# Audio-WestlakeU/FS-EEND

Measured on AMD Instinct MI355X. Metric: audio frames/sec (T=500 chunks), higher is better.
Workload: dtype bf16

## Files before the change

### fs-eend_amd/csrc/api.hip

```cpp
#include "../../include/eend_hip.h"
#include "kernels.h"
#include <stdlib.h>
#include <string.h>

namespace {
GemmParams base_params(const void* A, int lda, const void* W, int ldw, const float* bias, int M, int N, int K) {
    GemmParams p;
    memset(&p, 0, sizeof(p));
    p.A = A; p.lda = lda; p.W = W; p.ldw = ldw; p.bias = bias;
    p.M = M; p.N = N; p.K = K; p.ldo = N; p.Tp = 64; p.H = 4; p.dh = 64; p.C = 1;
    p.alpha = 1.0f; p.eps = 1e-5f; p.conv_cin = 64; p.conv_pad = 0; p.drop.scale = 1.0f;
#ifdef EEND_GEMM_ABLATE
    const char* d = getenv("EEND_GEMM_DBG");
    p.dbg = d ? atoi(d) : 0;
#endif
    return p;
}

hipStream_t hs(void* stream) { return (hipStream_t)stream; }

bool linear_takes_proj(int act, const float* bias, int ldw, int ldo, int N, int K) {
    return act == 0 && K == 256 && ldw == 256 && bias && (N % 256) == 0 && N <= 1024 && (ldo & 7) == 0;
}
bool heads_shape_ok(int nseq, int Tp, int H, int dh) {
// ... 708 lines not shown
int eend_inproj_attn_packed_elems(void) { return (int)eend_inproj_attn_packed_nelems(); }

int eend_inproj_attn_pack_f16(const void* W_in, void* packed_out, void* stream) {
    return eend_launch_inproj_attn_pack(W_in, packed_out, (hipStream_t)stream);
}

int eend_inproj_attn_causal_packed_f16(const void* X_f16, int ldx, const void* W_packed, const float* b_in, void* O_f16,
                                       int nseq, int H, int Tp, int ldo, int mask_delay, int kv_len, void* stream) {
    if (!X_f16 || !W_packed || !b_in || !O_f16 || nseq > 16383) return EEND_EINVAL;
    InprojAttnParams p;
    p.X = X_f16; p.ldx = ldx; p.W = W_packed; p.bias = b_in; p.O = O_f16;
    p.nseq = nseq; p.H = H; p.Tp = Tp; p.ldo = ldo; p.mask_delay = mask_delay; p.kv_len = kv_len;
    return eend_launch_inproj_attn_stream(p, (hipStream_t)stream);
}

int eend_inproj_attn_long_scratch_elems(int nseq, int Tp, int mask_delay, int kv_len, long long* part_f16_elems, long long* lse_f32_elems) {
    if (!part_f16_elems || !lse_f32_elems) return EEND_EINVAL;
    long a = 0, b = 0;
    const int rc = eend_inproj_attn_long_scratch(nseq, Tp, mask_delay, kv_len, &a, &b);
    *part_f16_elems = a; *lse_f32_elems = b;
    return rc;
}

int eend_inproj_attn_causal_long_f16(const void* X_f16, int ldx, const void* W_packed, const float* b_in, void* O_f16, void* part_f16,
                                     float* lse_f32, int nseq, int H, int Tp, int ldo, int mask_delay, int kv_len, void* stream) {
    if (!X_f16 || !W_packed || !b_in || !O_f16 || !lse_f32 || nseq > 16383) return EEND_EINVAL;
    InprojAttnParams p;
    memset(&p, 0, sizeof(p));
    p.X = X_f16; p.ldx = ldx; p.W = W_packed; p.bias = b_in; p.O = O_f16; p.Opart = part_f16; p.lse = lse_f32;
    p.nseq = nseq; p.H = H; p.Tp = Tp; p.ldo = ldo; p.mask_delay = mask_delay; p.kv_len = kv_len;
// ... 168 lines not shown
```

### fs-eend_amd/csrc/attn_stream.hip

```cpp
#include "flash_tile.h"
#include "kernels.h"
#include "wstream.h"
#include <stdlib.h>

namespace {

constexpr int KB = 64;
constexpr int TILE = KB * 128;
constexpr int NW = 8;
constexpr int OSTG = 32 * 128;
constexpr int TP = 512;
constexpr int NT = TP / KB;
constexpr int WITEM = 16384;
constexpr int NITEM = 6;
constexpr int L_K = 0, L_V = NT * TILE, L_X = 2 * NT * TILE;
constexpr int SMEM = L_X + NW * OSTG;

DEV u32x2 pack_bf16x4(const f32x4 v) {
    bf16x4 o;
    o[0] = (__bf16)v[0]; o[1] = (__bf16)v[1]; o[2] = (__bf16)v[2]; o[3] = (__bf16)v[3];
    return __builtin_bit_cast(u32x2, o);
}

__global__ void inproj_attn_pack_kernel(const _Float16* __restrict__ W, _Float16* __restrict__ out) {
// ... 3 lines not shown
        const int pfrag = w >> 6, l = w & 63, f = l & 15, g = l >> 4, ks = pfrag >> 1, hf = pfrag & 1;
        const _Float16* src = W + (size_t)((n >> 1) * 256 + h * 64 + ((n & 1) * 2 + hf) * 16 + f) * 256 + ks * 32 + g * 8;
        _Float16* dst = out + (size_t)t * 8;
#pragma unroll
        for (int e = 0; e < 8; ++e) dst[e] = src[e];
    }
}

#ifdef EEND_AS_TRACE
__device__ unsigned long long g_as_trace[256 * 6 * 12];
#define AS_STAMP(k) do { ts[k] = __builtin_amdgcn_s_memtime(); } while (0)
#else
#define AS_STAMP(k) do {} while (0)
#endif

template <bool LONG, bool TRAIN = false, bool FULL = false>
__global__ __launch_bounds__(512)
void inproj_attn_stream_kernel(const InprojAttnParams p) {
    static_assert(!(LONG && TRAIN), "the training form covers windows up to 512 frames");
    static_assert(!(LONG && FULL), "groups of a long window have their own lengths");
    extern __shared__ __attribute__((aligned(16))) char smem[];
    char* Ks = smem + L_K;
    char* Vs = smem + L_V;
    char* Xs = smem + L_X;

    int tid = threadIdx.x;
    int lane = tid & 63;
    const int wave = __builtin_amdgcn_readfirstlane(tid >> 6);
    int frow = lane & 15, fkg = lane >> 4;
    const int nsh = p.nseq * 4;
    const int nitems = LONG ? nsh * p.npairs : nsh;
    const bool xcd_map = (p.nseq & 7) == 0 && ((gridDim.x & 7) == 0 || (int)gridDim.x >= nitems);
    auto item_of = [&](int L, int& seq_, int& h_) __attribute__((always_inline)) {
        if (xcd_map) {
            const int xcd = L & 7, slot = L >> 3;
            seq_ = (slot >> 2) * 8 + xcd; h_ = slot & 3;
        } else {
            seq_ = L >> 2; h_ = L & 3;
        }
    };
    int nblk = FULL ? 16 : p.Tp >> 5;
    int b1 = FULL ? wave : (wave < (nblk >> 1) ? wave : nblk + 2 * (wave - (nblk >> 1)));
    int b2 = FULL ? 15 - wave : (wave < (nblk >> 1) ? nblk - 1 - wave : b1 + 1);
    int qoff = 0, koff = 0, Tq = p.Tp, Tk = p.Tp, dl = p.mask_delay, kvl = p.kv_len, pair = 0;
    bool offd = false;
    auto tokbase = [&](int jt) __attribute__((always_inline)) { return jt < 2 ? 32 * b1 + 16 * jt : 32 * b2 + 16 * (jt - 2); };
    char* Ow = Xs + wave * OSTG;
    auto relaunder = [&]() __attribute__((always_inline)) {
        asm volatile("" : "+v"(tid));
        lane = tid & 63; frow = lane & 15; fkg = lane >> 4;
    };

    u32x4 xr[4][8];
    auto request_x = [&](int seq_, auto KEYS) __attribute__((always_inline)) {
        constexpr bool keys = decltype(KEYS)::value;
        const __amdgpu_buffer_rsrc_t rx = __builtin_amdgcn_make_buffer_rsrc((void*)((const _Float16*)p.X + ((size_t)seq_ * p.Tp + (keys ? koff : qoff)) * p.ldx), 0,
                                                                            (keys ? Tk : Tq) * p.ldx * 2, 0x00020000);
#pragma unroll
        for (int jt = 0; jt < 4; ++jt) {
// ... 6 lines not shown
    for (int item = blockIdx.x; item < nitems; item += gridDim.x) {
    int seq, h;
    if constexpr (LONG) {
        pair = item / nsh;
        item_of(item - pair * nsh, seq, h);
        const int qg = p.pq[pair], kg = p.pk[pair];
        qoff = qg * TP; koff = kg * TP;
        Tq = p.Tp - qoff < TP ? p.Tp - qoff : TP;
        Tk = p.Tp - koff < TP ? p.Tp - koff : TP;
        offd = qg != kg;
        dl = p.mask_delay + (qoff - koff);
        kvl = p.kv_len - koff < Tk ? p.kv_len - koff : Tk;
        nblk = Tq >> 5;
        b1 = wave < (nblk >> 1) ? wave : nblk + 2 * (wave - (nblk >> 1));
        b2 = wave < (nblk >> 1) ? nblk - 1 - wave : b1 + 1;
    } else {
        item_of(item, seq, h);
    }
    relaunder();
    request_x(seq, std::false_type{});
    asm volatile("s_waitcnt lgkmcnt(0)\n\ts_barrier" ::: "memory");
#ifdef EEND_AS_TRACE
    unsigned long long ts[12];
    const int tix = (item - (int)blockIdx.x) / (int)gridDim.x;
#endif
    AS_STAMP(0);

    u32x2 qpk[4][4];
    {
        const __amdgpu_buffer_rsrc_t rw = __builtin_amdgcn_make_buffer_rsrc((void*)((const char*)p.W + (size_t)h * NITEM * WITEM), 0,
                                                                            NITEM * WITEM, 0x00020000);
        f32x4 bq4[4];
        float bv1[4];
        f32x4 bk4[TRAIN ? 4 : 1], bv4[TRAIN ? 4 : 1];
#pragma unroll
        for (int ff = 0; ff < 4; ++ff) {
            const float4 t4 = *(const float4*)(p.bias + h * 64 + ff * 16 + fkg * 4);
            bq4[ff] = f32x4{t4.x, t4.y, t4.z, t4.w};
            bv1[ff] = p.bias[512 + h * 64 + ff * 16 + frow];
            if constexpr (TRAIN) {
                const float4 k4 = *(const float4*)(p.bias + 256 + h * 64 + ff * 16 + fkg * 4);
                const float4 v4 = *(const float4*)(p.bias + 512 + h * 64 + ff * 16 + fkg * 4);
                bk4[ff] = f32x4{k4.x, k4.y, k4.z, k4.w};
                bv4[ff] = f32x4{v4.x, v4.y, v4.z, v4.w};
            }
        }
#pragma unroll
        for (int n = 0; n < NITEM; ++n) {
            char* dst = n < 4 ? Vs + n * WITEM : Xs + (n - 4) * WITEM;
#pragma unroll
            for (int i = 0; i < 2; ++i)
                __builtin_amdgcn_raw_ptr_buffer_load_lds(rw, (lds_char*)(dst + (wave * 2 + i) * 1024), 16, lane * 16,
                                                         n * WITEM + (wave * 2 + i) * 1024, 0, 0);
        }
        f16x8 x[4][8];
        auto rows_to_fragments = [&]() __attribute__((always_inline)) {
            char* xt = Ks + wave * 8192;
#pragma unroll
            for (int jt = 0; jt < 4; ++jt) {
#pragma unroll
                for (int i = 0; i < 8; ++i) {
                    const int r = 2 * i + (lane >> 5);
                    *(u32x4*)(xt + r * 512 + (((lane & 31) ^ r) << 4)) = xr[jt][i];
                }
                wave_lds_sync();
#pragma unroll
                for (int ks = 0; ks < 8; ++ks) x[jt][ks] = __builtin_bit_cast(f16x8, *(const u32x4*)(xt + frow * 512 + (((ks * 4 + fkg) ^ frow) << 4)));
                wave_lds_sync();
            }
        };
        rows_to_fragments();
        sfor<NITEM>([&](auto N) __attribute__((always_inline)) {
            constexpr int n = decltype(N)::value, kind = n >> 1, ffb = (n & 1) * 2;
            if constexpr (LONG && n == 2) {
                if (offd) {
                    relaunder();
                    request_x(seq, std::true_type{});
                    rows_to_fragments();
                }
            }
            wait_vm<2 * (NITEM - 1 - n)>();
            __builtin_amdgcn_s_barrier();
            AS_STAMP(1 + n);
            relaunder();
            const char* wi = smem + lane * 16 + (n < 4 ? L_V + n * WITEM : L_X + (n - 4) * WITEM);
            f32x4 acc[2][4];
            f32x4 accv[TRAIN && kind == 2 ? 2 : 1][4];
#pragma unroll
            for (int hf = 0; hf < 2; ++hf) {
                f32x4 b4 = f32x4{0.f, 0.f, 0.f, 0.f};
                if constexpr (kind == 2) b4 = f32x4{bv1[ffb + hf], bv1[ffb + hf], bv1[ffb + hf], bv1[ffb + hf]};
                else if constexpr (kind == 0) b4 = bq4[ffb + hf];
                else if constexpr (TRAIN) b4 = bk4[ffb + hf];
#pragma unroll
                for (int jt = 0; jt < 4; ++jt) {
                    acc[hf][jt] = b4;
                    if constexpr (TRAIN && kind == 2) accv[hf][jt] = bv4[ffb + hf];
                }
            }
            constexpr int NB = 8, PD = 4;
// ... 16 lines not shown
            });
#pragma unroll
            for (int hf = 0; hf < 2; ++hf)
#pragma unroll
                for (int jt = 0; jt < 4; ++jt) {
                    const u32x2 v = pack_bf16x4(acc[hf][jt]);
                    if constexpr (TRAIN) {
                        const int tok = tokbase(jt) + frow;
                        if (tok < p.Tp) {
                            __bf16* dst = (__bf16*)(kind == 0 ? p.Qh : kind == 1 ? p.Kh : p.Vh) + (((size_t)(seq * 4 + h) * p.Tp + tok) * 64 + (ffb + hf) * 16 + fkg * 4);
                            if constexpr (kind == 2) *(u32x2*)dst = pack_bf16x4(accv[hf][jt]);
                            else *(u32x2*)dst = v;
                        }
                    }
                    if constexpr (kind == 0) {
                        qpk[ffb + hf][jt] = v;
                    } else if constexpr (kind == 1) {
                        const int key = (LONG && offd ? 64 * wave + 16 * jt : tokbase(jt)) + frow, d = (ffb + hf) * 16 + fkg * 4;
                        *(u32x2*)(Ks + (key >> 6) * TILE + swz128(key & 63, d >> 3) + (d & 7) * 2) = v;
                    } else {
                        const int d = (ffb + hf) * 16 + frow, key = (LONG && offd ? 64 * wave + 16 * jt : tokbase(jt)) + fkg * 4;
                        *(u32x2*)(Vs + (key >> 6) * TILE + swz128(d, (key & 63) >> 3) + (key & 7) * 2) = v;
                    }
                }
        });
        AS_STAMP(7);
        asm volatile("s_waitcnt vmcnt(0) lgkmcnt(0)\n\ts_barrier" ::: "memory");
        AS_STAMP(8);
    }

    relaunder();
    const int lq = lane & 31, hi = lane >> 5;
    const int krow = swap23(lq);

    bf16x8 qf[4];
    f32x16 oT[2];
    f32x16 mneg;
    float l_run;
    int qw0, q;

    auto begin_pass = [&](int qb, auto JT0) __attribute__((always_inline)) {
        constexpr int jt0 = decltype(JT0)::value;
        qw0 = qb * 32;
        q = qw0 + lq;
        stage_packed(Ow, frow, fkg, qpk, jt0);
        staged_operand(Ow, lq, hi, qf);
#pragma unroll
        for (int i = 0; i < 16; ++i) { oT[0][i] = 0.f; oT[1][i] = 0.f; mneg[i] = 0.f; }
        l_run = 0.f;
    };
    auto tile = [&](int j) __attribute__((always_inline)) {
        const int key0 = j * KB;
        const char* kb_ = Ks + j * TILE;
        const char* vb_ = Vs + j * TILE;
        f32x16 s[2];
#pragma unroll
        for (int kb = 0; kb < 2; ++kb)
#pragma unroll
            for (int ks = 0; ks < 4; ++ks) {
                const bf16x8 kf = *(const bf16x8*)(kb_ + swz128(kb * 32 + krow, ks * 2 + hi));
// ... 17 lines not shown
    };
    auto run_pass = [&](int qb, auto JT0) __attribute__((always_inline)) {
        begin_pass(qb, JT0);
        int last_key = qw0 + 31 + dl;
        last_key = last_key < kvl - 1 ? last_key : kvl - 1;
        const int jend = last_key < 0 ? 0 : last_key / KB + 1;
        for (int j = 0; j < jend; ++j) tile(j);
        const float l_tot = l_run + __shfl_xor(l_run, 32, 64);
        const float inv = LONG ? (l_tot > 0.f ? 1.0f / l_tot : 0.f) : 1.0f / l_tot;
        if constexpr (LONG) {
            if (hi == 0) p.lse[((size_t)(pair * p.nseq + seq) * 4 + h) * TP + q] = l_tot > 0.f ? __builtin_amdgcn_logf(l_tot) - mneg[0] : -1e30f;
        }
        if constexpr (TRAIN) {
            if (hi == 0) p.lse[(size_t)(seq * 4 + h) * p.Tp + q] = __builtin_amdgcn_logf(l_tot) - mneg[0];
        }
        stage_rows(Ow, lq, hi, [&](int db, int i) __attribute__((always_inline)) { return to_f16_sat(oT[db][i] * inv); });
        _Float16* __restrict__ Og = (_Float16*)p.O + ((size_t)seq * p.Tp + qoff + qw0) * p.ldo + h * 64;
        int ldo = p.ldo;
        if constexpr (LONG) {
            if (offd) { Og = (_Float16*)p.Opart + ((size_t)(p.pslot[pair] * p.nseq + seq) * TP + qw0) * 256 + h * 64; ldo = 256; }
        }
        store_staged_rows(Ow, lane, Og, ldo);
    };
    if (FULL || b2 < nblk) run_pass(b2, std::integral_constant<int, 2>{});
    AS_STAMP(9);
    if (FULL || b1 < nblk) run_pass(b1, std::integral_constant<int, 0>{});
    AS_STAMP(10);
    AS_STAMP(11);
#ifdef EEND_AS_TRACE
    if (tix < 6 && threadIdx.x == 0) {
#pragma unroll
        for (int k = 0; k < 12; ++k) g_as_trace[((size_t)blockIdx.x * 6 + tix) * 12 + k] = ts[k];
    }
#endif
    }
}

__global__ __launch_bounds__(256)
void attn_long_combine_kernel(const InprojAttnParams p) {
    const int row = blockIdx.x * 8 + (threadIdx.x >> 5);
    const int seq = blockIdx.y;
    if (row >= p.Tp) return;
// ... 50 lines not shown
int eend_launch_inproj_attn_stream(const InprojAttnParams& p, hipStream_t stream) {
    if (p.Tp <= 0 || p.Tp > TP || (p.Tp & 63) || (p.ldo & 7) || (p.ldx & 7) || p.H != 4 || p.nseq <= 0 || !p.X || !p.W || !p.bias || !p.O ||
        p.kv_len < 1 || p.kv_len > p.Tp)
        return EEND_EINVAL;
    static EendOncePerDevice attr_once;
    static EendOncePerDevice attr_once_full;
    if (!eend_set_dynamic_lds(attr_once, (const void*)inproj_attn_stream_kernel<false, false, false>, SMEM)) return EEND_ELAUNCH;
    if (!eend_set_dynamic_lds(attr_once_full, (const void*)inproj_attn_stream_kernel<false, false, true>, SMEM)) return EEND_ELAUNCH;
    int n_cu = eend_cu_count() & ~31;
    if (n_cu <= 0) n_cu = 32;
    const int nitems = p.nseq * 4;
    InprojAttnParams q = p;
    q.npairs = 0; q.Opart = nullptr; q.lse = nullptr;
    if (p.Tp == TP) hipLaunchKernelGGL((inproj_attn_stream_kernel<false, false, true>), dim3(nitems < n_cu ? nitems : n_cu), dim3(512), SMEM, stream, q);
    else hipLaunchKernelGGL((inproj_attn_stream_kernel<false, false, false>), dim3(nitems < n_cu ? nitems : n_cu), dim3(512), SMEM, stream, q);
    return hipGetLastError() == hipSuccess ? EEND_OK : EEND_ELAUNCH;
}

int eend_launch_inproj_attn_train(const InprojAttnParams& p, hipStream_t stream) {
    if (p.Tp <= 0 || p.Tp > TP || (p.Tp & 63) || (p.ldo & 7) || (p.ldx & 7) || p.H != 4 || p.nseq <= 0 || !p.X || !p.W || !p.bias || !p.O || !p.Qh || !p.Kh ||
        !p.Vh || !p.lse || p.kv_len < 1 || p.kv_len > p.Tp || (long)p.nseq * 4 * p.Tp >= (1L << 31))
        return EEND_EINVAL;
    static EendOncePerDevice attr_once;
    static EendOncePerDevice attr_once_full;
    if (!eend_set_dynamic_lds(attr_once, (const void*)inproj_attn_stream_kernel<false, true, false>, SMEM)) return EEND_ELAUNCH;
    if (!eend_set_dynamic_lds(attr_once_full, (const void*)inproj_attn_stream_kernel<false, true, true>, SMEM)) return EEND_ELAUNCH;
    int n_cu = eend_cu_count() & ~31;
    if (n_cu <= 0) n_cu = 32;
    const int nitems = p.nseq * 4;
    InprojAttnParams q = p;
// ... 61 lines not shown
```

### fs-eend_amd/csrc/kernels.h

```cpp
#pragma once
#include <hip/hip_runtime.h>
#include <stdint.h>
#include "../../include/eend_hip.h"
#include "common.h"

enum GemmEpilogue {
    EPI_PLAIN_F16 = 0,
    EPI_PLAIN_RELU_F16 = 1,
    EPI_QK_HEADS = 2,
    EPI_VT_HEADS = 3,
    EPI_RES_LN = 4,
    EPI_L2NORM = 5,
    EPI_CONVERT = 6,
    EPI_RES_SCALE = 7,
    EPI_RES_SCALE_LN16 = 8,
    EPI_PLAIN_SWISH_F16 = 9,
    EPI_GLU_F16 = 10,
    EPI_QK_HEADS_F16 = 11,
    EPI_KTVT_HEADS_F16 = 12,
    EPI_PLAIN_BF16 = 13,
    EPI_MASK_BF16 = 14,
    EPI_F32_ROWMASK = 15,
    EPI_RES_LN_TRAIN = 16,
    EPI_L2NORM_TRAIN = 17,
// ... 131 lines not shown
int eend_launch_gemm(const GemmParams& p, int epi, hipStream_t stream, int* route = nullptr);

#define EEND_ATTN_LONG_MAX_PAIRS 64
struct InprojAttnParams {
    const void* X; int ldx;
    const void* W;
    const float* bias;
    void* O;
    int nseq, H, Tp, ldo, mask_delay, kv_len;
    int npairs;
    void* Opart;
    float* lse;
    unsigned char pq[EEND_ATTN_LONG_MAX_PAIRS], pk[EEND_ATTN_LONG_MAX_PAIRS], pslot[EEND_ATTN_LONG_MAX_PAIRS];
    void* Qh; void* Kh; void* Vh;
    DropSpec drop;
};
int eend_launch_inproj_attn_train(const InprojAttnParams& p, hipStream_t stream);
long eend_inproj_attn_packed_nelems();
int eend_inproj_attn_long_scratch(int nseq, int Tp, int mask_delay, int kv_len, long* part_elems, long* lse_elems);
int eend_launch_inproj_attn_long(const InprojAttnParams& p, hipStream_t stream);
int eend_launch_inproj_attn_pack(const void* W, void* out, hipStream_t stream);
int eend_launch_inproj_attn_stream(const InprojAttnParams& p, hipStream_t stream);

#define EEND_SKINNY_MAX_M 16
bool eend_skinny_ok(const void* A, int lda, const void* W, int ldw, int M, int K);
int eend_launch_skinny_plain(const void* A, int lda, const void* W, int ldw, const float* bias, void* out16, int ldo,
                             int M, int N, int K, int act, hipStream_t stream, int* route = nullptr);
int eend_launch_skinny_glu(const void* A, int lda, const void* W, int ldw, const float* bias, void* out16, int ldo,
                           int M, int N2, int K, hipStream_t stream, int* route = nullptr);
int eend_launch_skinny_res(const void* A, int lda, const void* W, int ldw, const float* bias, const float* res, float alpha,
                           const float* gamma, const float* beta, float eps, float* out32, void* out16, int M, int K,
// ... 418 lines not shown
```

### fs-eend_amd/fs_model.py

```python
import copy
import math
from typing import List, Optional, Sequence

import torch
import torch.nn as nn
from torch import Tensor

from . import ops
from .lib import EendHipError

_D_SUPPORTED = 256
_H_SUPPORTED = 4


class PositionalEncoding(nn.Module):

    def __init__(self, d_model, dropout=0.1, max_len=5000):
        super().__init__()
        self.dropout = nn.Dropout(p=dropout)
        pe = torch.zeros(max_len, d_model)
        position = torch.arange(0, max_len, dtype=torch.float).unsqueeze(1)
        div_term = torch.exp(torch.arange(0, d_model, 2).float() * (-math.log(10000.0) / d_model))
        pe[:, 0::2] = torch.sin(position * div_term)
        pe[:, 1::2] = torch.cos(position * div_term)
# ... 137 lines not shown
        super().__init__()
        if n_units != _D_SUPPORTED or n_heads != _H_SUPPORTED:
            raise NotImplementedError("HIP kernels are specialised for n_units=256, n_heads=4 (all reference configs)")
        self.n_speakers = n_speakers
        self.delay = conv_delay
        self.enc = MaskedTransformerEncoderModel(in_size, n_heads, n_units, enc_n_layers, dropout=dropout,
                                                 has_mask=has_mask, max_seqlen=max_seqlen, mask_delay=mask_delay)
        self.dec = MaskedTransformerDecoderModel(in_size, n_heads, n_units, dec_n_layers,
                                                 dim_feedforward=dec_dim_feedforward, dropout=dropout,
                                                 has_mask=has_mask, max_seqlen=max_seqlen, mask_delay=mask_delay)
        self.cnn = nn.Conv1d(n_units, n_units, kernel_size=2 * conv_delay + 1, padding=9)
        self._prep = None
        self._prep_key = None
        self._ws = WorkspaceCache()
        self._pc = {}
        self.register_load_state_dict_post_hook(lambda module, incompatible_keys: module.refresh_weights())

    def refresh_weights(self):
        self._prep = None

    def _apply(self, fn, *a, **kw):
        out = super()._apply(fn, *a, **kw)
        self._prep = None
        return out

    def _fingerprint(self):
        return tuple((p.data_ptr(), p._version) for p in list(self.parameters()) + list(self.buffers()))

    def _prepare(self):
        key = self._fingerprint()
# ... 44 lines not shown
                out2_w=_f16(l.self_attn2.out_proj.weight), out2_b=_f32(l.self_attn2.out_proj.bias),
                w1=_f16(l.linear1.weight), b1=_f32(l.linear1.bias), w2=_f16(l.linear2.weight), b2=_f32(l.linear2.bias),
                g11=_f32(l.norm11.weight), be11=_f32(l.norm11.bias), eps11=l.norm11.eps,
                g21=_f32(l.norm21.weight), be21=_f32(l.norm21.bias), eps21=l.norm21.eps,
                g22=_f32(l.norm22.weight), be22=_f32(l.norm22.bias), eps22=l.norm22.eps))
        for L in dl:
            if ops.stream_ok(L["w1"].shape[0]):
                L["ws"] = ops.ffn_stream_pack(L["out2_w"], L["w1"], L["w2"])
            L["ws1"] = ops.spk_stream_pack(L["out1_w"], L["in2_w"])
            if ops.stream_ok(L["w1"].shape[0]):
                L["wsd"] = ops.dec_stream_pack(L["out1_w"], L["in2_w"], L["out2_w"], L["w1"], L["w2"])
            L["in1_wp"] = ops.inproj_attn_pack(L["in1_w"])
        P["dec.layers"] = dl
        self._prep, self._prep_key = P, key
        self._pc = {}
        return P

    def _convert_const(self, C):
        if C not in self._pc:
            from . import lib as _lib
            D = self.enc.n_units if hasattr(self.enc, "n_units") else self.n_units
            dev = self.dec.convert.weight.device
            W = self.dec.convert.weight.detach().to(torch.float32).contiguous()
            b = self.dec.convert.bias.detach().to(torch.float32).contiguous()
            pe = self.dec.pos_enc.pe[0, :C].to(device=dev, dtype=torch.float32).contiguous()
            pc = torch.empty(C, D, dtype=torch.float32, device=dev)
            L = _lib.load()
            _lib.check(L.eend_convert_const_f32(0, W.data_ptr(), b.data_ptr(), pe.data_ptr(), pc.data_ptr(), None, None, None, C,
                                                torch.cuda.current_stream().cuda_stream), "eend_convert_const_f32")
            self._pc[C] = pc
        return self._pc[C]

    def _workspace(self, dev, B, Tp, C):
        key = (str(dev), B, Tp, C)
        ws = self._ws.get(key)
        if ws is None:
            P = self._prep
            F_enc = P["enc.layers"][0]["w1"].shape[0] if P["enc.layers"] else 0
            F_dec = P["dec.layers"][0]["w1"].shape[0] if P["dec.layers"] else 0
            ws = _Workspace(dev, B, Tp, C, self.enc.n_units, F_enc, F_dec, P["Fin_pad"], self.enc.n_heads)
            self._ws.put(key, ws)
        return ws

    def _run(self, src: Sequence[Tensor], ilens: Sequence[int], C: int):
        P = self._prepare()
        dev = self.cnn.weight.device
# ... 7 lines not shown
            ws.il = torch.tensor(il_key, dtype=torch.int32, device=dev)
            ws.il_key = il_key
        il = ws.il
        Me, Md = B * Tp, B * C * Tp
        delay_e = self.enc.mask_delay if self.enc.has_mask else Tp
        kv_e = T

        if ops.encoder_input_ok(srcs, Tp, P["enc.in.w"]):
            ops.encoder_input(srcs, P["bn"], P["enc.in.w"], P["enc.in.b"], P["enc.in.g"], P["enc.in.beta"], None, ws.h16, T, Tp, -1.0,
                              P["bn.eps"], P["enc.in.eps"])
        else:
            ops.gather_bn_cast_pad(srcs, P["bn"], ws.xin16, T, Tp, -1.0, True, P["bn.eps"])
            ops.linear_res_ln(ws.xin16, P["enc.in.w"], P["enc.in.b"], None, P["enc.in.g"], P["enc.in.beta"], None, ws.h16, P["enc.in.eps"])
        o16 = ws.o16[:Me]

        def time_attention(x16, Ly, wkey, bkey, nseq, delay, kv):
            o = ws.o16[:nseq * Tp]
            if Tp <= 512:
                ops.inproj_attn_causal_packed(x16, Ly[wkey + "p"], Ly[bkey], o, nseq, H, Tp, delay, kv)
                return o
            need = ops.inproj_attn_long_scratch(nseq, Tp, delay, kv) if Tp <= 3072 else None
            if need is not None:
                if ws.attn_part.numel() < need[0]:
                    ws.attn_part = torch.empty(need[0], dtype=torch.float16, device=o.device)
                if ws.attn_lse.numel() < need[1]:
                    ws.attn_lse = torch.empty(need[1], dtype=torch.float32, device=o.device)
                ops.inproj_attn_causal_long(x16, Ly[wkey + "p"], Ly[bkey], o, ws.attn_part, ws.attn_lse, nseq, H, Tp, delay, kv)
            else:
                n = nseq * Tp * D
                if ws.q is None:
                    ws.q, ws.k, ws.vt = (torch.empty(ws.Mx * ws.D, dtype=torch.bfloat16, device=o.device) for _ in range(3))
                ops.inproj_heads(x16, Ly[wkey], Ly[bkey], ws.q[:n], ws.k[:n], ws.vt[:n], nseq, Tp, H)
# ... 5 lines not shown
            if "ws" in L:
                ops.attnout_ffn_stream(o16, L["ws"], L["out_b"], None, ws.h16, L["g1"], L["be1"], L["eps1"], L["b1"], L["b2"], L["g2"],
                                       L["be2"], L["eps2"], None, ws.h16)
            else:
                ops.attnout_ffn_fused_res16(o16, L["out_w"], L["out_b"], ws.h16, L["g1"], L["be1"], L["eps1"], L["w1"], L["b1"],
                                            L["w2"], L["b2"], L["g2"], L["be2"], L["eps2"], None, ws.h16)

        emb32 = torch.empty(Me, D, dtype=torch.float32, device=dev)
        if "cnn.ws" in P:
            ops.conv1d_l2norm_stream(ws.h16, P["cnn.ws"], P["cnn.b"], il, emb32, ws.emb16, B, Tp, P["cnn.k"], P["cnn.pad"])
        else:
            ops.conv1d_l2norm(ws.h16, P["cnn.w"], P["cnn.b"], il, emb32, ws.emb16, B, Tp, D, P["cnn.k"], P["cnn.pad"])

        ops.convert_fanout(ws.emb16, P["convert.w1"], self._convert_const(C), None, ws.a16, B, Tp, C)
        o16 = ws.o16[:Md]
        for L in P["dec.layers"]:
            time_attention(ws.a16, L, "in1_w", "in1_b", B * C, self.dec.mask_delay, T)
            if "wsd" in L and ops.dec_stream_ok(C, Tp):
                ops.attnout_spk_ffn_stream(o16, L["wsd"], L["out1_b"], ws.a16, L["g11"], L["be11"], L["eps11"], L["in2_b"], L["out2_b"],
                                           L["g21"], L["be21"], L["eps21"], L["b1"], L["b2"], L["g22"], L["be22"], L["eps22"], ws.a16, B, C, Tp)
                continue
            ops.attnout_spk_stream(o16, L["ws1"], L["out1_b"], ws.a16, L["g11"], L["be11"], L["eps11"], ws.a16, L["in2_b"], o16, B, C, Tp)
            if "ws" in L:
                ops.attnout_ffn_stream(o16, L["ws"], L["out2_b"], None, ws.a16, L["g21"], L["be21"], L["eps21"], L["b1"], L["b2"],
                                       L["g22"], L["be22"], L["eps22"], None, ws.a16)
            else:
                ops.attnout_ffn_fused_res16(o16, L["out2_w"], L["out2_b"], ws.a16, L["g21"], L["be21"], L["eps21"], L["w1"], L["b1"],
                                            L["w2"], L["b2"], L["g22"], L["be22"], L["eps22"], None, ws.a16)

        attr = torch.empty(B, T, C, D, dtype=torch.float32, device=dev)
        logits = torch.empty(B, T, C, dtype=torch.float32, device=dev)
        ops.head_l2dot(emb32, ws.a16, attr, logits, B, T, Tp, C, D)
# ... 27 lines not shown
```

### fs-eend_amd/lib.py

```python
import ctypes
import os

_HERE = os.path.dirname(os.path.abspath(__file__))
LIB_PATH = os.environ.get("EEND_HIP_LIB") or os.path.join(_HERE, "csrc", "libeend_hip.so")

_vp, _i, _f = ctypes.c_void_p, ctypes.c_int, ctypes.c_float
_l = ctypes.c_long

ABI_VERSION = 5

PROTOTYPES = {
    "eend_abi_version": [],
    "eend_bn_cast_pad_f16": [_vp, _vp, _vp, _vp, _vp, _f, _vp, _i, _i, _i, _i, _i, _i, _vp],
    "eend_gather_bn_cast_pad_f16": [_vp, _vp, _f, _vp, _vp, _vp, _vp, _f, _vp, _i, _i, _i, _i, _i, _i, _vp],
    "eend_linear_f16": [_vp, _i, _vp, _i, _vp, _vp, _i, _i, _i, _i, _i, _vp],
    "eend_inproj_heads_bf16": [_vp, _i, _vp, _i, _vp, _vp, _vp, _vp, _i, _i, _i, _i, _i, _vp],
    "eend_linear_glu_f16": [_vp, _i, _vp, _i, _vp, _vp, _i, _i, _i, _i, _vp],
    "eend_linear_res_ln_f16": [_vp, _i, _vp, _i, _vp, _vp, _f, _vp, _vp, _f, _vp, _vp, _i, _i, _vp],
    "eend_linear_res16_ln_f16": [_vp, _i, _vp, _i, _vp, _vp, _f, _vp, _vp, _f, _vp, _vp, _i, _i, _vp],
    "eend_linear_res_scale_ln16_f16": [_vp, _i, _vp, _i, _vp, _vp, _f, _vp, _vp, _f, _vp, _vp, _i, _i, _vp],
    "eend_ffn_fused_f16": [_vp, _i, _vp, _vp, _vp, _vp, _vp, _f, _vp, _vp, _f, _vp, _vp, _i, _i, _i, _i, _vp],
    "eend_attnout_ffn_fused_f16": [_vp, _i, _vp, _vp, _vp, _vp, _vp, _f, _vp, _vp, _vp, _vp, _vp, _vp, _f, _vp, _vp, _vp, _vp, _i, _i, _vp],
    "eend_attnout_ffn_fused_res16_f16": [_vp, _i, _vp, _vp, _vp, _vp, _vp, _f, _vp, _vp, _vp, _vp, _vp, _vp, _f, _vp, _vp, _i, _i, _vp],
    "eend_convert_fanout_f32": [_vp, _vp, _i, _vp, _vp, _vp, _vp, _i, _i, _i, _vp],
    "eend_ffn_stream_elems": [_i, _i],
    "eend_ffn_stream_pack_f16": [_vp, _vp, _vp, _vp, _i, _vp],
    "eend_ffn_stream_pack_lo_f16": [_vp, _vp, _vp, _vp, _vp, _i, _vp],
    "eend_attnout_ffn_stream_lo_f16": [_vp, _i, _vp, _vp, _vp, _vp, _vp, _f, _vp, _vp, _vp, _vp, _f, _vp, _vp, _vp, _i, _i, _vp],
    "eend_ffn_stream_f16": [_vp, _i, _vp, _vp, _vp, _vp, _f, _vp, _vp, _f, _vp, _vp, _i, _i, _i, _i, _vp],
    "eend_conv_stream_elems": [_i],
    "eend_conv_stream_ok": [_i, _i, _i],
    "eend_conv_stream_pack_f16": [_vp, _vp, _i, _vp],
    "eend_conv1d_l2norm_stream_f16": [_vp, _vp, _vp, _vp, _vp, _vp, _i, _i, _i, _i, _vp],
    "eend_encoder_input_ok": [_i, _i, _i],
    "eend_encoder_input_f16": [_vp, _vp, _f, _vp, _vp, _vp, _vp, _f, _vp, _i, _vp, _vp, _vp, _f, _vp, _vp, _i, _i, _i, _i, _vp],
    "eend_inproj_attn_packed_elems": [],
    "eend_inproj_attn_pack_f16": [_vp, _vp, _vp],
    "eend_inproj_attn_causal_packed_f16": [_vp, _i, _vp, _vp, _vp, _i, _i, _i, _i, _i, _i, _vp],
    "eend_inproj_attn_train_bf16": [_vp, _i, _vp, _vp, _vp, _i, _vp, _vp, _vp, _vp, _i, _i, _i, _i, _i, _vp, _vp],
    "eend_gemm_acc_stream_elems": [_i],
    "eend_gemm_acc_stream_ok": [_i, _i, _i],
    "eend_gemm_acc_stream_pack_bf16": [_vp, _i, _vp, _i, _vp],
    "eend_gemm_acc_stream_bf16": [_vp, _i, _vp, _vp, _i, _i, _vp],
    "eend_proj_stream_elems": [_i],
    "eend_proj_stream_pack_f16": [_vp, _vp, _i, _vp],
    "eend_proj_stream_ok": [_i, _i, _i, _i, _i, _vp],
    "eend_proj_stream_f16": [_vp, _i, _vp, _vp, _i, _i, _i, _i, _vp, _vp],
    "eend_inproj_attn_long_scratch_elems": [_i, _i, _i, _i, _vp, _vp],
    "eend_inproj_attn_causal_long_f16": [_vp, _i, _vp, _vp, _vp, _vp, _vp, _i, _i, _i, _i, _i, _i, _vp],
    "eend_spk_stream_elems": [],
    "eend_spk_stream_ok": [_i, _i],
    "eend_spk_stream_pack_f16": [_vp, _vp, _vp, _vp],
    "eend_attnout_spk_stream_f16": [_vp, _i, _vp, _vp, _vp, _vp, _vp, _f, _vp, _vp, _vp, _i, _i, _i, _f, _vp],
# ... 220 lines not shown
```

### fs-eend_amd/ops.py

```python
import math

import torch

from . import lib as _lib

F16, BF16, F32 = torch.float16, torch.bfloat16, torch.float32


def _stream():
    return torch.cuda.current_stream().cuda_stream


def _p(t):
    return None if t is None else t.data_ptr()


def _chk(t, dtype, name):
    if t is None:
        return
    if not t.is_cuda:
        raise _lib.EendHipError(f"{name}: expected a GPU tensor (the HIP path has no CPU fallback)")
    if t.dtype != dtype:
        raise _lib.EendHipError(f"{name}: expected {dtype}, got {t.dtype}")
    if not t.is_contiguous():
# ... 240 lines not shown
    _chk(q, BF16, "q"); _chk(k, BF16, "k"); _chk(vt, BF16, "vt"); _chk(o16, F16, "o16")
    _lib.check(L.eend_attn_causal_bf16(_p(q), _p(k), _p(vt), _p(o16), nseq, H, Tp, o16.stride(0), mask_delay,
                                       Tp if kv_len is None else kv_len, scale, _stream()), "eend_attn_causal_bf16")


def inproj_attn_pack(w_in):
    L = _lib.load()
    _chk(w_in, F16, "w_in")
    if w_in.shape != (768, 256):
        raise _lib.EendHipError("inproj_attn_pack: expected in_proj_weight [768][256]")
    out = torch.empty(L.eend_inproj_attn_packed_elems(), dtype=F16, device=w_in.device)
    _lib.check(L.eend_inproj_attn_pack_f16(_p(w_in), _p(out), _stream()), "eend_inproj_attn_pack_f16")
    return out


def inproj_attn_causal_packed(x16, w_packed, b_in, o16, nseq, H, Tp, mask_delay=0, kv_len=None):
    L = _lib.load()
    _chk(x16, F16, "x16"); _chk(w_packed, F16, "w_packed"); _chk(b_in, F32, "b_in"); _chk(o16, F16, "o16")
    if w_packed.numel() != L.eend_inproj_attn_packed_elems() or b_in.numel() != 768 or x16.shape[0] < nseq * Tp or o16.shape[0] < nseq * Tp:
        raise _lib.EendHipError("inproj_attn_causal_packed: shape mismatch")
    _lib.check(L.eend_inproj_attn_causal_packed_f16(_p(x16), x16.stride(0), _p(w_packed), _p(b_in), _p(o16), nseq, H, Tp,
                                                    o16.stride(0), mask_delay, Tp if kv_len is None else kv_len, _stream()),
               "eend_inproj_attn_causal_packed_f16")


def inproj_attn_long_scratch(nseq, Tp, mask_delay=0, kv_len=None):
    import ctypes
    L = _lib.load()
    a, b = ctypes.c_longlong(0), ctypes.c_longlong(0)
    rc = L.eend_inproj_attn_long_scratch_elems(nseq, Tp, mask_delay, Tp if kv_len is None else kv_len, ctypes.byref(a), ctypes.byref(b))
    return None if rc != 0 else (a.value, b.value)


def inproj_attn_causal_long(x16, w_packed, b_in, o16, part16, lse32, nseq, H, Tp, mask_delay=0, kv_len=None):
    L = _lib.load()
# ... 780 lines not shown
```

### include/eend_hip.h

```cpp
#ifndef EEND_HIP_H
#define EEND_HIP_H

#ifdef __cplusplus
extern "C" {
#endif

#define EEND_OK 0
#define EEND_EINVAL (-1)
#define EEND_ELAUNCH (-2)

#define EEND_ABI_VERSION 5
int eend_abi_version(void);

int eend_bn_cast_pad_f16(const float* x, const float* bn_weight, const float* bn_bias,
                         const float* bn_mean, const float* bn_var, float eps, void* out_f16,
                         int B, int T, int Tp, int Fin, int Fpad, int apply_bn, void* stream);

int eend_gather_bn_cast_pad_f16(const void* const* x_ptrs, const int* lens, float pad_value,
                                const float* bn_weight, const float* bn_bias, const float* bn_mean,
                                const float* bn_var, float eps, void* out_f16, int B, int T, int Tp, int Fin,
                                int Fpad, int apply_bn, void* stream);

int eend_encoder_input_ok(int Fin, int Tp, int ldw);
int eend_encoder_input_f16(const float* const* x_ptrs, const int* lens, float pad_value, const float* bn_w, const float* bn_b,
// ... 251 lines not shown
int eend_convert_fanout_step_f32(const float* emb_f32, const float* W_f32, int ldw, const float* pc, float* out_f32, void* out_f16,
                                 int B, int C, void* stream);

int eend_dwconv_step_f16(const void* x_f16, float* cache, const float* w, const float* bn_weight,
                         const float* bn_bias, const float* bn_mean, const float* bn_var, float eps,
                         void* out_f16, int B, int D, int k, void* stream);

int eend_spk_attn_f16(const void* qkv, void* O_f16, int B, int C, int Tp, int H, float scale,
                      void* stream);


int eend_inproj_attn_packed_elems(void);
int eend_inproj_attn_pack_f16(const void* W_in, void* packed_out, void* stream);
int eend_inproj_attn_causal_packed_f16(const void* X_f16, int ldx, const void* W_packed, const float* b_in, void* O_f16,
                                       int nseq, int H, int Tp, int ldo, int mask_delay, int kv_len, void* stream);

int eend_inproj_attn_long_scratch_elems(int nseq, int Tp, int mask_delay, int kv_len, long long* part_f16_elems, long long* lse_f32_elems);
int eend_inproj_attn_causal_long_f16(const void* X_f16, int ldx, const void* W_packed, const float* b_in, void* O_f16, void* part_f16,
                                     float* lse_f32, int nseq, int H, int Tp, int ldo, int mask_delay, int kv_len, void* stream);


int eend_head_l2dot_f32(const float* emb, const float* attr, float* attr_out, float* logits, int B, int T,
                        int Tp, int C, int D, void* stream);
int eend_head_l2dot_a16_f32(const float* emb, const void* attr_f16, float* attr_out, float* logits, int B, int T,
                            int Tp, int C, int D, void* stream);



typedef struct eend_dropout {
    unsigned seed;
// ... 217 lines not shown
```

Measured before the change: 16.78 million.

## Share first decoder layer attention projection across speaker slots via per-slot deltas

```diff
diff --git a/fs-eend_amd/csrc/api.hip b/fs-eend_amd/csrc/api.hip
--- a/fs-eend_amd/csrc/api.hip
+++ b/fs-eend_amd/csrc/api.hip
@@ -746,6 +746,23 @@
     return eend_launch_inproj_attn_stream(p, (hipStream_t)stream);
 }
 
+int eend_inproj_attn_slots_choice(int n_utt, int C, int workgroups) {
+    const int S = eend_attn_slots_choice(n_utt, C, workgroups);
+    return S > 0 ? S : EEND_EINVAL;
+}
+
+int eend_inproj_attn_causal_slots_f16(const void* X_f16, int ldx, const void* W_packed, const float* b_in, void* O_f16,
+                                      int nseq, int H, int Tp, int ldo, int mask_delay, int kv_len, int C, const float* slot_delta,
+                                      int slots_per_item, void* stream) {
+    if (!X_f16 || !W_packed || !b_in || !O_f16 || nseq > 16383) return EEND_EINVAL;
+    InprojAttnParams p;
+    memset(&p, 0, sizeof(p));
+    p.X = X_f16; p.ldx = ldx; p.W = W_packed; p.bias = b_in; p.O = O_f16;
+    p.nseq = nseq; p.H = H; p.Tp = Tp; p.ldo = ldo; p.mask_delay = mask_delay; p.kv_len = kv_len;
+    p.C = C; p.slot_delta = slot_delta; p.S = slots_per_item;
+    return eend_launch_inproj_attn_slots(p, (hipStream_t)stream);
+}
+
 int eend_inproj_attn_long_scratch_elems(int nseq, int Tp, int mask_delay, int kv_len, long long* part_f16_elems, long long* lse_f32_elems) {
     if (!part_f16_elems || !lse_f32_elems) return EEND_EINVAL;
     long a = 0, b = 0;
diff --git a/fs-eend_amd/csrc/attn_stream.hip b/fs-eend_amd/csrc/attn_stream.hip
--- a/fs-eend_amd/csrc/attn_stream.hip
+++ b/fs-eend_amd/csrc/attn_stream.hip
@@ -41,11 +41,12 @@
 #define AS_STAMP(k) do {} while (0)
 #endif
 
-template <bool LONG, bool TRAIN = false, bool FULL = false>
+template <bool LONG, bool TRAIN = false, bool FULL = false, bool SLOTS = false>
 __global__ __launch_bounds__(512)
 void inproj_attn_stream_kernel(const InprojAttnParams p) {
     static_assert(!(LONG && TRAIN), "the training form covers windows up to 512 frames");
     static_assert(!(LONG && FULL), "groups of a long window have their own lengths");
+    static_assert(!SLOTS || (FULL && !TRAIN), "the slot form exists for inference at 512 frames");
     extern __shared__ __attribute__((aligned(16))) char smem[];
     char* Ks = smem + L_K;
     char* Vs = smem + L_V;
@@ -55,9 +56,10 @@
     int lane = tid & 63;
     const int wave = __builtin_amdgcn_readfirstlane(tid >> 6);
     int frow = lane & 15, fkg = lane >> 4;
-    const int nsh = p.nseq * 4;
-    const int nitems = LONG ? nsh * p.npairs : nsh;
-    const bool xcd_map = (p.nseq & 7) == 0 && ((gridDim.x & 7) == 0 || (int)gridDim.x >= nitems);
+    const int nsq = SLOTS ? p.nutt : p.nseq;
+    const int nsh = nsq * 4;
+    const int nitems = LONG ? nsh * p.npairs : SLOTS ? nsh * p.ngrp : nsh;
+    const bool xcd_map = (nsq & 7) == 0 && ((gridDim.x & 7) == 0 || (int)gridDim.x >= nitems);
     auto item_of = [&](int L, int& seq_, int& h_) __attribute__((always_inline)) {
         if (xcd_map) {
             const int xcd = L & 7, slot = L >> 3;
@@ -70,6 +72,7 @@
     int b1 = FULL ? wave : (wave < (nblk >> 1) ? wave : nblk + 2 * (wave - (nblk >> 1)));
     int b2 = FULL ? 15 - wave : (wave < (nblk >> 1) ? nblk - 1 - wave : b1 + 1);
     int qoff = 0, koff = 0, Tq = p.Tp, Tk = p.Tp, dl = p.mask_delay, kvl = p.kv_len, pair = 0;
+    int c0 = 0, oseq = 0;
     bool offd = false;
     auto tokbase = [&](int jt) __attribute__((always_inline)) { return jt < 2 ? 32 * b1 + 16 * jt : 32 * b2 + 16 * (jt - 2); };
     char* Ow = Xs + wave * OSTG;
@@ -106,6 +109,11 @@
         nblk = Tq >> 5;
         b1 = wave < (nblk >> 1) ? wave : nblk + 2 * (wave - (nblk >> 1));
         b2 = wave < (nblk >> 1) ? nblk - 1 - wave : b1 + 1;
+    } else if constexpr (SLOTS) {
+        const int grp = item / nsh;
+        item_of(item - grp * nsh, seq, h);
+        c0 = grp * p.S;
+        seq *= p.C;
     } else {
         item_of(item, seq, h);
     }
@@ -118,7 +126,19 @@
 #endif
     AS_STAMP(0);
 
-    u32x2 qpk[4][4];
+    f32x4 dq[SLOTS ? 4 : 1];
+    float dv1 = 0.f;
+    auto slot_rsrc = [&](int c, int cend) __attribute__((always_inline)) {
+        return __builtin_amdgcn_make_buffer_rsrc((void*)(p.slot_delta + (size_t)c * 512), 0, c > 0 && c < cend ? 2048 : 0, 0x00020000);
+    };
+    auto load_dq = [&](int c, int cend, f32x4 (&d)[SLOTS ? 4 : 1]) __attribute__((always_inline)) {
+        const __amdgpu_buffer_rsrc_t rd = slot_rsrc(c, cend);
+#pragma unroll
+        for (int ff = 0; ff < (SLOTS ? 4 : 1); ++ff)
+            d[ff] = __builtin_bit_cast(f32x4, __builtin_amdgcn_raw_buffer_load_b128(rd, (h * 64 + ff * 16 + fkg * 4) * 4, 0, 0));
+    };
+    u32x2 qpk[SLOTS ? 1 : 4][4];
+    f32x4 qacc[SLOTS ? 4 : 1][4];
     {
         const __amdgpu_buffer_rsrc_t rw = __builtin_amdgcn_make_buffer_rsrc((void*)((const char*)p.W + (size_t)h * NITEM * WITEM), 0,
                                                                             NITEM * WITEM, 0x00020000);
@@ -137,14 +157,14 @@
                 bv4[ff] = f32x4{v4.x, v4.y, v4.z, v4.w};
             }
         }
-#pragma unroll
-        for (int n = 0; n < NITEM; ++n) {
-            char* dst = n < 4 ? Vs + n * WITEM : Xs + (n - 4) * WITEM;
+        auto request_w = [&](int n, char* dst) __attribute__((always_inline)) {
 #pragma unroll
             for (int i = 0; i < 2; ++i)
                 __builtin_amdgcn_raw_ptr_buffer_load_lds(rw, (lds_char*)(dst + (wave * 2 + i) * 1024), 16, lane * 16,
                                                          n * WITEM + (wave * 2 + i) * 1024, 0, 0);
-        }
+        };
+#pragma unroll
+        for (int n = SLOTS ? 2 : 0; n < NITEM; ++n) request_w(n, n < 4 ? Vs + n * WITEM : Xs + (n - 4) * WITEM);
         f16x8 x[4][8];
         auto rows_to_fragments = [&]() __attribute__((always_inline)) {
             char* xt = Ks + wave * 8192;
@@ -163,7 +183,8 @@
         };
         rows_to_fragments();
         sfor<NITEM>([&](auto N) __attribute__((always_inline)) {
-            constexpr int n = decltype(N)::value, kind = n >> 1, ffb = (n & 1) * 2;
+            constexpr int m = decltype(N)::value, n = SLOTS ? (m + 2) % NITEM : m;
+            constexpr int kind = n >> 1, ffb = (n & 1) * 2;
             if constexpr (LONG && n == 2) {
                 if (offd) {
                     relaunder();
@@ -171,11 +192,12 @@
                     rows_to_fragments();
                 }
             }
-            wait_vm<2 * (NITEM - 1 - n)>();
+            wait_vm<SLOTS ? (m < 3 ? 2 * (3 - m) : 0) : 2 * (NITEM - 1 - n)>();
             __builtin_amdgcn_s_barrier();
-            AS_STAMP(1 + n);
+            AS_STAMP(1 + m);
             relaunder();
-            const char* wi = smem + lane * 16 + (n < 4 ? L_V + n * WITEM : L_X + (n - 4) * WITEM);
+            if constexpr (SLOTS && (m == 3 || m == 4)) request_w(m - 3, Xs + (m - 3) * WITEM);
+            const char* wi = smem + lane * 16 + (SLOTS && n < 2 ? L_X + n * WITEM : n < 4 ? L_V + n * WITEM : L_X + (n - 4) * WITEM);
             f32x4 acc[2][4];
             f32x4 accv[TRAIN && kind == 2 ? 2 : 1][4];
 #pragma unroll
@@ -222,7 +244,8 @@
                         }
                     }
                     if constexpr (kind == 0) {
-                        qpk[ffb + hf][jt] = v;
+                        if constexpr (SLOTS) qacc[ffb + hf][jt] = acc[hf][jt];
+                        else qpk[ffb + hf][jt] = v;
                     } else if constexpr (kind == 1) {
                         const int key = (LONG && offd ? 64 * wave + 16 * jt : tokbase(jt)) + frow, d = (ffb + hf) * 16 + fkg * 4;
                         *(u32x2*)(Ks + (key >> 6) * TILE + swz128(key & 63, d >> 3) + (d & 7) * 2) = v;
@@ -232,14 +255,15 @@
                     }
                 }
         });
+        if constexpr (SLOTS) load_dq(c0, c0 + p.S, dq);
         AS_STAMP(7);
         asm volatile("s_waitcnt vmcnt(0) lgkmcnt(0)\n\ts_barrier" ::: "memory");
         AS_STAMP(8);
     }
 
     relaunder();
-    const int lq = lane & 31, hi = lane >> 5;
-    const int krow = swap23(lq);
+    int lq = lane & 31, hi = lane >> 5;
+    int krow = swap23(lq);
 
     bf16x8 qf[4];
     f32x16 oT[2];
@@ -251,7 +275,17 @@
         constexpr int jt0 = decltype(JT0)::value;
         qw0 = qb * 32;
         q = qw0 + lq;
-        stage_packed(Ow, frow, fkg, qpk, jt0);
+        if constexpr (SLOTS) {
+            u32x2 qs[4][2];
+#pragma unroll
+            for (int ff = 0; ff < 4; ++ff)
+#pragma unroll
+                for (int jl = 0; jl < 2; ++jl) qs[ff][jl] = pack_bf16x4(qacc[ff][jt0 + jl] + dq[ff]);
+            load_dq(oseq - seq + (jt0 == 2 ? 0 : 1), c0 + p.S, dq);
+            stage_packed(Ow, frow, fkg, qs, 0);
+        } else {
+            stage_packed(Ow, frow, fkg, qpk, jt0);
+        }
         staged_operand(Ow, lq, hi, qf);
 #pragma unroll
         for (int i = 0; i < 16; ++i) { oT[0][i] = 0.f; oT[1][i] = 0.f; mneg[i] = 0.f; }
@@ -299,18 +333,39 @@
         if constexpr (TRAIN) {
             if (hi == 0) p.lse[(size_t)(seq * 4 + h) * p.Tp + q] = __builtin_amdgcn_logf(l_tot) - mneg[0];
         }
-        stage_rows(Ow, lq, hi, [&](int db, int i) __attribute__((always_inline)) { return to_f16_sat(oT[db][i] * inv); });
-        _Float16* __restrict__ Og = (_Float16*)p.O + ((size_t)seq * p.Tp + qoff + qw0) * p.ldo + h * 64;
+        if constexpr (SLOTS) {
+            stage_rows(Ow, lq, hi, [&](int db, int i) __attribute__((always_inline)) { 
+                const int feat = db * 32 + (i >> 2) * 8 + hi * 4 + (i & 3);
+                return to_f16_sat(oT[db][i] * inv + __builtin_bit_cast(float, __builtin_amdgcn_ds_bpermute(feat << 2, __builtin_bit_cast(int, dv1))));
+            });
+        } else {
+            stage_rows(Ow, lq, hi, [&](int db, int i) __attribute__((always_inline)) { return to_f16_sat(oT[db][i] * inv); });
+        }
+        _Float16* __restrict__ Og = (_Float16*)p.O + ((size_t)(SLOTS ? oseq : seq) * p.Tp + qoff + qw0) * p.ldo + h * 64;
         int ldo = p.ldo;
         if constexpr (LONG) {
             if (offd) { Og = (_Float16*)p.Opart + ((size_t)(p.pslot[pair] * p.nseq + seq) * TP + qw0) * 256 + h * 64; ldo = 256; }
         }
         store_staged_rows(Ow, lane, Og, ldo);
     };
+    if constexpr (SLOTS) {
+        for (int c = c0; c < c0 + p.S; ++c) {
+            oseq = seq + c;
+            relaunder();
+            lq = lane & 31; hi = lane >> 5; krow = swap23(lq);
+            const __amdgpu_buffer_rsrc_t rd = slot_rsrc(c, c0 + p.S);
+            dv1 = __builtin_bit_cast(float, __builtin_amdgcn_raw_buffer_load_b32(rd, (256 + h * 64 + lane) * 4, 0, 0));
+            run_pass(b2, std::integral_constant<int, 2>{});
+            AS_STAMP(9);
+            run_pass(b1, std::integral_constant<int, 0>{});
+            AS_STAMP(10);
+        }
+    } else {
     if (FULL || b2 < nblk) run_pass(b2, std::integral_constant<int, 2>{});
     AS_STAMP(9);
     if (FULL || b1 < nblk) run_pass(b1, std::integral_constant<int, 0>{});
     AS_STAMP(10);
+    }
     AS_STAMP(11);
 #ifdef EEND_AS_TRACE
     if (tix < 6 && threadIdx.x == 0) {
@@ -391,6 +446,38 @@
     q.npairs = 0; q.Opart = nullptr; q.lse = nullptr;
     if (p.Tp == TP) hipLaunchKernelGGL((inproj_attn_stream_kernel<false, false, true>), dim3(nitems < n_cu ? nitems : n_cu), dim3(512), SMEM, stream, q);
     else hipLaunchKernelGGL((inproj_attn_stream_kernel<false, false, false>), dim3(nitems < n_cu ? nitems : n_cu), dim3(512), SMEM, stream, q);
+    return hipGetLastError() == hipSuccess ? EEND_OK : EEND_ELAUNCH;
+}
+
+int eend_attn_slots_choice(int nutt, int C, int workgroups) {
+    if (nutt < 1 || C < 1 || C > 12 || workgroups < 1) return 0;
+    constexpr long T_FIX = 231, T_SLOT = 341;
+    int best = 1;
+    long best_cost = -1;
+    for (int S = 1; S <= C; ++S) {
+        if (C % S) continue;
+        const long items = 4L * nutt * (C / S);
+        const long cost = ((items + workgroups - 1) / workgroups) * (T_FIX + S * T_SLOT);
+        if (best_cost < 0 || cost < best_cost) { best = S; best_cost = cost; }
+    }
+    return best;
+}
+
+int eend_launch_inproj_attn_slots(const InprojAttnParams& p, hipStream_t stream) {
+    if (p.Tp != TP || (p.ldo & 7) || (p.ldx & 7) || p.H != 4 || p.nseq <= 0 || !p.X || !p.W || !p.bias || !p.O || p.kv_len < 1 || p.kv_len > p.Tp ||
+        p.C < 1 || p.C > 12 || p.nseq % p.C || (p.C > 1 && !p.slot_delta) || p.S < 0 || (p.S > 0 && p.C % p.S))
+        return EEND_EINVAL;
+    static EendOncePerDevice attr_once;
+    if (!eend_set_dynamic_lds(attr_once, (const void*)inproj_attn_stream_kernel<false, false, true, true>, SMEM)) return EEND_ELAUNCH;
+    int n_cu = eend_cu_count() & ~31;
+    if (n_cu <= 0) n_cu = 32;
+    InprojAttnParams q = p;
+    q.npairs = 0; q.Opart = nullptr; q.lse = nullptr;
+    q.nutt = p.nseq / p.C;
+    if (q.S == 0) q.S = eend_attn_slots_choice(q.nutt, p.C, n_cu);
+    q.ngrp = p.C / q.S;
+    const int nitems = q.nutt * 4 * q.ngrp;
+    hipLaunchKernelGGL((inproj_attn_stream_kernel<false, false, true, true>), dim3(nitems < n_cu ? nitems : n_cu), dim3(512), SMEM, stream, q);
     return hipGetLastError() == hipSuccess ? EEND_OK : EEND_ELAUNCH;
 }
 
diff --git a/fs-eend_amd/csrc/kernels.h b/fs-eend_amd/csrc/kernels.h
--- a/fs-eend_amd/csrc/kernels.h
+++ b/fs-eend_amd/csrc/kernels.h
@@ -169,7 +169,11 @@
     unsigned char pq[EEND_ATTN_LONG_MAX_PAIRS], pk[EEND_ATTN_LONG_MAX_PAIRS], pslot[EEND_ATTN_LONG_MAX_PAIRS];
     void* Qh; void* Kh; void* Vh;
     DropSpec drop;
-};
+    int C, S, nutt, ngrp;
+    const float* slot_delta;
+};
+int eend_attn_slots_choice(int nutt, int C, int workgroups);
+int eend_launch_inproj_attn_slots(const InprojAttnParams& p, hipStream_t stream);
 int eend_launch_inproj_attn_train(const InprojAttnParams& p, hipStream_t stream);
 long eend_inproj_attn_packed_nelems();
 int eend_inproj_attn_long_scratch(int nseq, int Tp, int mask_delay, int kv_len, long* part_elems, long* lse_elems);
diff --git a/fs-eend_amd/fs_model.py b/fs-eend_amd/fs_model.py
--- a/fs-eend_amd/fs_model.py
+++ b/fs-eend_amd/fs_model.py
@@ -175,6 +175,7 @@
         self._prep_key = None
         self._ws = WorkspaceCache()
         self._pc = {}
+        self._sd = {}
         self.register_load_state_dict_post_hook(lambda module, incompatible_keys: module.refresh_weights())
 
     def refresh_weights(self):
@@ -249,6 +250,7 @@
         P["dec.layers"] = dl
         self._prep, self._prep_key = P, key
         self._pc = {}
+        self._sd = {}
         return P
 
     def _convert_const(self, C):
@@ -265,6 +267,16 @@
                                                 torch.cuda.current_stream().cuda_stream), "eend_convert_const_f32")
             self._pc[C] = pc
         return self._pc[C]
+
+    def _slot_delta(self, C):
+        if C not in self._sd:
+            W = self._prep["dec.layers"][0]["in1_w"].to(torch.float32)
+            pc = self._convert_const(C)
+            d = pc - pc[:1]
+            sd = (d[:, None, :] * torch.cat([W[:256], W[512:]])[None]).sum(-1)
+            sd[0] = 0.0
+            self._sd[C] = sd.contiguous()
+        return self._sd[C]
 
     def _workspace(self, dev, B, Tp, C):
         key = (str(dev), B, Tp, C)
@@ -302,8 +314,12 @@
             ops.linear_res_ln(ws.xin16, P["enc.in.w"], P["enc.in.b"], None, P["enc.in.g"], P["enc.in.beta"], None, ws.h16, P["enc.in.eps"])
         o16 = ws.o16[:Me]
 
-        def time_attention(x16, Ly, wkey, bkey, nseq, delay, kv):
+        def time_attention(x16, Ly, wkey, bkey, nseq, delay, kv, slots=None):
             o = ws.o16[:nseq * Tp]
+            if slots is not None and Tp == 512:
+                ops.inproj_attn_causal_packed(x16, Ly[wkey + "p"], Ly[bkey], o, nseq, H, Tp, delay, kv, slots=slots,
+                                              slot_delta=self._slot_delta(slots))
+                return o
             if Tp <= 512:
                 ops.inproj_attn_causal_packed(x16, Ly[wkey + "p"], Ly[bkey], o, nseq, H, Tp, delay, kv)
                 return o
@@ -339,8 +355,8 @@
 
         ops.convert_fanout(ws.emb16, P["convert.w1"], self._convert_const(C), None, ws.a16, B, Tp, C)
         o16 = ws.o16[:Md]
-        for L in P["dec.layers"]:
-            time_attention(ws.a16, L, "in1_w", "in1_b", B * C, self.dec.mask_delay, T)
+        for li, L in enumerate(P["dec.layers"]):
+            time_attention(ws.a16, L, "in1_w", "in1_b", B * C, self.dec.mask_delay, T, slots=C if li == 0 and C <= 12 else None)
             if "wsd" in L and ops.dec_stream_ok(C, Tp):
                 ops.attnout_spk_ffn_stream(o16, L["wsd"], L["out1_b"], ws.a16, L["g11"], L["be11"], L["eps11"], L["in2_b"], L["out2_b"],
                                            L["g21"], L["be21"], L["eps21"], L["b1"], L["b2"], L["g22"], L["be22"], L["eps22"], ws.a16, B, C, Tp)
diff --git a/fs-eend_amd/lib.py b/fs-eend_amd/lib.py
--- a/fs-eend_amd/lib.py
+++ b/fs-eend_amd/lib.py
@@ -37,6 +37,8 @@
     "eend_inproj_attn_packed_elems": [],
     "eend_inproj_attn_pack_f16": [_vp, _vp, _vp],
     "eend_inproj_attn_causal_packed_f16": [_vp, _i, _vp, _vp, _vp, _i, _i, _i, _i, _i, _i, _vp],
+    "eend_inproj_attn_slots_choice": [_i, _i, _i],
+    "eend_inproj_attn_causal_slots_f16": [_vp, _i, _vp, _vp, _vp, _i, _i, _i, _i, _i, _i, _i, _vp, _i, _vp],
     "eend_inproj_attn_train_bf16": [_vp, _i, _vp, _vp, _vp, _i, _vp, _vp, _vp, _vp, _i, _i, _i, _i, _i, _vp, _vp],
     "eend_gemm_acc_stream_elems": [_i],
     "eend_gemm_acc_stream_ok": [_i, _i, _i],
diff --git a/fs-eend_amd/ops.py b/fs-eend_amd/ops.py
--- a/fs-eend_amd/ops.py
+++ b/fs-eend_amd/ops.py
@@ -278,11 +278,29 @@
     return out
 
 
-def inproj_attn_causal_packed(x16, w_packed, b_in, o16, nseq, H, Tp, mask_delay=0, kv_len=None):
+def inproj_attn_slots_choice(n_utt, C, workgroups):
+    S = _lib.load().eend_inproj_attn_slots_choice(n_utt, C, workgroups)
+    if S < 1:
+        _lib.check(S, "eend_inproj_attn_slots_choice")
+    return S
+
+
+def inproj_attn_causal_packed(x16, w_packed, b_in, o16, nseq, H, Tp, mask_delay=0, kv_len=None, *, slots=None, slot_delta=None,
+                              slots_per_item=0):
     L = _lib.load()
     _chk(x16, F16, "x16"); _chk(w_packed, F16, "w_packed"); _chk(b_in, F32, "b_in"); _chk(o16, F16, "o16")
     if w_packed.numel() != L.eend_inproj_attn_packed_elems() or b_in.numel() != 768 or x16.shape[0] < nseq * Tp or o16.shape[0] < nseq * Tp:
         raise _lib.EendHipError("inproj_attn_causal_packed: shape mismatch")
+    if slots is not None:
+        if slot_delta is not None:
+            _chk(slot_delta, F32, "slot_delta")
+            if slot_delta.numel() < slots * 512:
+                raise _lib.EendHipError("inproj_attn_causal_packed: slot_delta must hold [slots][512]")
+        _lib.check(L.eend_inproj_attn_causal_slots_f16(_p(x16), x16.stride(0), _p(w_packed), _p(b_in), _p(o16), nseq, H, Tp,
+                                                       o16.stride(0), mask_delay, Tp if kv_len is None else kv_len, slots,
+                                                       _p(slot_delta), slots_per_item, _stream()),
+                   "eend_inproj_attn_causal_slots_f16")
+        return
     _lib.check(L.eend_inproj_attn_causal_packed_f16(_p(x16), x16.stride(0), _p(w_packed), _p(b_in), _p(o16), nseq, H, Tp,
                                                     o16.stride(0), mask_delay, Tp if kv_len is None else kv_len, _stream()),
                "eend_inproj_attn_causal_packed_f16")
diff --git a/include/eend_hip.h b/include/eend_hip.h
--- a/include/eend_hip.h
+++ b/include/eend_hip.h
@@ -289,6 +289,11 @@
 int eend_inproj_attn_pack_f16(const void* W_in, void* packed_out, void* stream);
 int eend_inproj_attn_causal_packed_f16(const void* X_f16, int ldx, const void* W_packed, const float* b_in, void* O_f16,
                                        int nseq, int H, int Tp, int ldo, int mask_delay, int kv_len, void* stream);
+
+int eend_inproj_attn_slots_choice(int n_utt, int C, int workgroups);
+int eend_inproj_attn_causal_slots_f16(const void* X_f16, int ldx, const void* W_packed, const float* b_in, void* O_f16,
+                                      int nseq, int H, int Tp, int ldo, int mask_delay, int kv_len, int C, const float* slot_delta,
+                                      int slots_per_item, void* stream);
 
 int eend_inproj_attn_long_scratch_elems(int nseq, int Tp, int mask_delay, int kv_len, long long* part_f16_elems, long long* lse_f32_elems);
 int eend_inproj_attn_causal_long_f16(const void* X_f16, int ldx, const void* W_packed, const float* b_in, void* O_f16, void* part_f16,
```

New measurement: 17.26 million, median of 6. +2.9%, better.
